# lars-frogner/Impact

Measured on AMD Instinct MI355X. Metric: voxels stepped/sec + remesh tris/sec, 512^3 grid, 1/2/4/8 MI355X, higher is better.
Workload: dtype i8 voxels, f32 SDF/mesh arithmetic, f64 moments; 1 GPU; config-2 SDF asteroid x2.05 -> 502^3 grid = 512^3 stored voxels (32768 chunks); parallelism=single GPU, voxels_per_gpu=134217728, regions=1, triangles=1813104

## Files before the change

impact_amd/csrc/ivx_api.hip:

```cpp
#include <algorithm>
#include <array>
#include <functional>
#include <cmath>
#include <atomic>
#include <chrono>
#include <cstring>
#include <limits>
#include <map>
#include <unordered_map>
#include <new>
#include <vector>

#include <type_traits>

#include <dlfcn.h>

#include "ivx_internal.hpp"

static thread_local char g_error[512] = "";

void ivx_set_error(const char* fmt, ...) {
    va_list ap;
    va_start(ap, fmt);
    vsnprintf(g_error, sizeof(g_error), fmt, ap);
// ... 86 lines not shown
            block_release(g->mesh_block);
            g->mesh_block = nullptr;
        }
    }
}
int mesh_pool_assign(ivx_grid* const* grids, size_t n, const size_t* vcaps, const size_t* icaps, const size_t* scaps) {
    if (n == 0) return IVX_OK;
    auto up = [](size_t b) { return (b + 255) & ~(size_t)255; };
    size_t total = 0;
    for (size_t i = 0; i < n; ++i) total += 2 * up(vcaps[i] * 12) + up(vcaps[i] * 16) + up(icaps[i] * 4) + up(icaps[i] * 8) + up(scaps[i] * sizeof(ivx_submesh));
    ivx_block* blk = new (std::nothrow) ivx_block();
    IVX_REQUIRE(blk, IVX_ERR_CAPACITY, "mesh buffers: out of host memory");
    blk->dev = blk->pinned = nullptr;
    blk->refs = 0;
    if (hipMalloc(&blk->dev, total) != hipSuccess) {
        delete blk;
        ivx_set_error("mesh buffers: device allocation of %zu bytes for %zu objects failed", total, n);
        return IVX_ERR_HIP;
    }
    char* b = static_cast<char*>(blk->dev);
    for (size_t i = 0; i < n; ++i) {
        ivx_grid* g = grids[i];
        mesh_group_free(g, 1u), mesh_group_free(g, 2u), mesh_group_free(g, 4u);
        auto take = [&](auto*& p, size_t bytes) {
            p = reinterpret_cast<std::remove_reference_t<decltype(p)>>(b);
            b += up(bytes);
        };
        take(g->positions, vcaps[i] * 12), take(g->normals, vcaps[i] * 12), take(g->vertex_materials, vcaps[i] * 16);
        take(g->indices, icaps[i] * 4), take(g->index_materials, icaps[i] * 8), take(g->submeshes, scaps[i] * sizeof(ivx_submesh));
        g->vcap = vcaps[i], g->icap = icaps[i], g->scap = scaps[i];
        g->mesh_block = blk;
        g->mesh_pooled = 7u;
        g->mesh_generation += 1;
        blk->refs += 1;
    }
    return IVX_OK;
}

static int mesh_arena_mode() {
    static const int m = [] {
        const char* e = getenv("IVX_MESH_ARENA");
        return e ? atoi(e) : 0;
    }();
    return m;
}
static int ensure_mesh_block(ivx_grid* g, size_t nv, size_t ni) {
    if (nv <= g->vcap && ni <= g->icap) return IVX_OK;
    IVX_HIP_CHECK(ivx_stream_sync(g->ctx->stream));
    static const size_t phase = [] {
        const char* e = getenv("IVX_MESH_PHASE");
        return (size_t)(e ? strtoull(e, nullptr, 0) : 0ull);
    }();
    const size_t vcap = std::max(2 * nv + 4096, g->vcap * 2), icap = std::max(2 * ni + 24576, g->icap * 2);
    const size_t sizes[5] = {vcap * 12, vcap * 12, icap * 4, icap * 8, vcap * 16};
    size_t off[5], total = 0;
    for (int k = 0; k < 5; ++k) {
        total = (total + (2u << 20) - 1) & ~(size_t)((2u << 20) - 1);
        off[k] = total + (size_t)k * phase;
        total = off[k] + sizes[k];
    }
    mesh_group_free(g, 1u), mesh_group_free(g, 2u);
    g->vcap = g->icap = 0;
    ivx_block* blk = new (std::nothrow) ivx_block();
    IVX_REQUIRE(blk, IVX_ERR_CAPACITY, "mesh buffers: out of host memory");
    blk->dev = blk->pinned = nullptr;
    blk->refs = 1;
    if ((mesh_arena_mode() == 2 ? hipExtMallocWithFlags(&blk->dev, total, hipDeviceMallocContiguous) : hipMalloc(&blk->dev, total)) != hipSuccess) {
        delete blk;
        ivx_set_error("mesh buffers: device allocation of %zu bytes failed", total);
        return IVX_ERR_HIP;
    }
    char* b = static_cast<char*>(blk->dev);
    g->positions = reinterpret_cast<float*>(b + off[0]);
    g->normals = reinterpret_cast<float*>(b + off[1]);
    g->indices = reinterpret_cast<uint32_t*>(b + off[2]);
    g->index_materials = reinterpret_cast<uint8_t*>(b + off[3]);
    g->vertex_materials = reinterpret_cast<uint8_t*>(b + off[4]);
    g->vcap = vcap, g->icap = icap;
    if (g->mesh_block) block_release(g->mesh_block);
    g->mesh_block = blk;
    g->mesh_pooled = 3u;
    g->mesh_generation += 1;
    return IVX_OK;
}

int ensure_mesh_capacity(ivx_grid* g, size_t nv, size_t ni, size_t ns) {
    if (mesh_arena_mode())
        if (int rc = ensure_mesh_block(g, nv, ni)) return rc;
    if (nv > g->vcap || ni > g->icap || ns > g->scap) g->mesh_generation += 1;
    if (nv > g->vcap) {
        size_t cap = std::max(2 * nv + 4096, g->vcap * 2);
        mesh_group_free(g, 1u);
        g->vcap = 0;
        int rc;
        if ((rc = dev_alloc(&g->positions, cap * 3))) return rc;
        if ((rc = dev_alloc(&g->normals, cap * 3))) return rc;
        if ((rc = dev_alloc(&g->vertex_materials, cap * 16))) return rc;
        g->vcap = cap;
    }
    if (ni > g->icap) {
        size_t cap = std::max(2 * ni + 24576, g->icap * 2);
        mesh_group_free(g, 2u);
        g->icap = 0;
        int rc;
        if ((rc = dev_alloc(&g->indices, cap))) return rc;
        if ((rc = dev_alloc(&g->index_materials, cap * 8))) return rc;
        g->icap = cap;
    }
    if (ns > g->scap) {
        size_t cap = std::max(2 * ns + 64, g->scap * 2);
        mesh_group_free(g, 4u);
        g->scap = 0;
        int rc;
        if ((rc = dev_alloc(&g->submeshes, cap))) return rc;
        g->scap = cap;
    }
    return IVX_OK;
}

__global__ __launch_bounds__(256) void k_halo_pack(GridView g, uint32_t side, int8_t* __restrict__ out_sdf, uint8_t* __restrict__ out_type,
                                                   ivx_chunk_info* __restrict__ out_info) {
    const uint32_t col = blockIdx.x;
    const uint32_t tid = threadIdx.x;
    const uint32_t ci = side ? g.cx - 1 : 0u;
    const uint32_t chunk = ci * g.cy * g.cz + col;
// ... 251 lines not shown
        carve(&g->ghost_type[sd], cols * 256);
        carve(&g->ghost_info[sd], cols);
    }
    carve(&g->chunk_counts, (size_t)g->n_chunks * 2);
    carve(&g->chunk_offsets, (size_t)g->n_chunks * 3 + 8);
    carve(&g->partials, g->partial_blocks * 10 + 16);
    carve(&g->rparent, (size_t)g->n_chunks * 256);
    carve(&g->rcompid, (size_t)g->n_chunks * 256);
    carve(&g->rscalar, (size_t)64);
    carve(&g->ccl_scratch, (size_t)g->n_chunks * 2);
    carve(&g->sn_list, (size_t)g->n_chunks * 4);
    carve(&g->group_sums, (size_t)((g->n_chunks + 255u) / 256u) * (1u + IVX_SN_GROUP_WORDS) + IVX_SN_TAIL_WORDS);
    carve(&g->sn_hard, (size_t)g->n_chunks);
    carve(&g->sn_walk, (size_t)g->n_chunks * 5 + 2);
    carve(&g->dens_dev, (size_t)256);
    carve(&g->work_counts, (size_t)8);
    carve(&g->occ_part, (size_t)((g->n_chunks + 255u) / 256u) * 12 + 12);
    carve(&g->active_list, (size_t)g->n_chunks);
    carve(&g->chunk_class, (size_t)g->n_chunks);
    carve(&g->chunk_touch, (size_t)g->n_chunks);
    carve(&g->chunk_signs, (size_t)g->n_chunks * 256);
    carve(&g->kface, (size_t)g->n_chunks * 1024);
    carve(&g->chunk_moments, (size_t)g->n_chunks * 10);
    return arena_bytes;
}
static int grid_new(ivx_ctx* c, const uint32_t cc[3], float voxel_extent, uint32_t x_chunk_offset, uint32_t global_x_chunks, ivx_grid** out) {
    IVX_REQUIRE(c && cc && out, IVX_ERR_INVALID, "ivx_grid_create: null argument");
    *out = nullptr;
    IVX_REQUIRE(cc[0] > 0 && cc[1] > 0 && cc[2] > 0, IVX_ERR_INVALID, "ivx_grid_create: empty chunk grid");
    IVX_REQUIRE(voxel_extent > 0.0f, IVX_ERR_INVALID, "ivx_grid_create: voxel extent must be positive");
    const uint64_t n64 = (uint64_t)cc[0] * cc[1] * cc[2];
    IVX_REQUIRE(n64 <= (1u << 24), IVX_ERR_CAPACITY, "ivx_grid_create: more than 2^24 chunks");
    ivx_grid* g = new (std::nothrow) ivx_grid();
    IVX_REQUIRE(g, IVX_ERR_CAPACITY, "ivx_grid_create: out of host memory");
    memset(g, 0, sizeof(*g));
    g->scratch_dirty = IVX_SCRATCH_REGIONS;
    g->ctx = c;
    for (int d = 0; d < 3; ++d) g->cc[d] = cc[d];
    g->n_chunks = (uint32_t)n64;
    g->n_vox = (size_t)n64 * IVX_CHUNK_VOXELS;
    g->extent = voxel_extent;
    g->x_off = x_chunk_offset;
    g->gx = global_x_chunks ? global_x_chunks : cc[0];
    g->partial_blocks = 2048;
    *out = g;
    return IVX_OK;
}

static void ivx_block_release(ivx_block* b) { block_release(b); }

int ivx_grid_create(ivx_ctx* c, const uint32_t cc[3], float voxel_extent, uint32_t x_chunk_offset, uint32_t global_x_chunks, ivx_grid** out) {
    ivx_grid* g = nullptr;
    int rc = grid_new(c, cc, voxel_extent, x_chunk_offset, global_x_chunks, &g);
    if (rc) return rc;
    IVX_HIP_CHECK(hipSetDevice(c->device));
    const size_t arena_bytes = grid_carve(g, nullptr);
    char* arena = nullptr;
    if (hipMalloc(reinterpret_cast<void**>(&arena), arena_bytes) != hipSuccess) {
        ivx_set_error("ivx_grid_create: device allocation of %zu bytes failed", arena_bytes);
        delete g;
        return IVX_ERR_HIP;
    }
    g->arena = arena;
    (void)grid_carve(g, arena);
    if (ivx_memset_async(g->info, 0, sizeof(ivx_chunk_info) * g->n_chunks, c->stream) != hipSuccess ||
        ivx_memset_async(g->work_counts, 0, 8 * sizeof(uint32_t), c->stream) != hipSuccess) {
        ivx_set_error("ivx_grid_create: memset failed");
// ... 3215 lines not shown
```

impact_amd/csrc/ivx_internal.hpp:

```cpp
#pragma once
#include <hip/hip_runtime.h>

#include <cstdarg>
#include <cstdint>
#include <cstdio>
#include <cstring>

#include "../../include/impact_voxel_hip.h"
#include "many.hpp"

static inline hipError_t ivx_memset_async(void* p, int v, size_t n, hipStream_t s) {
    (void)ivx_many_break();
    return hipMemsetAsync(p, v, n, s);
}
static inline hipError_t ivx_memcpy_async(void* d, const void* src, size_t n, hipMemcpyKind k, hipStream_t s) {
    (void)ivx_many_break();
    return hipMemcpyAsync(d, src, n, k, s);
}
static inline hipError_t ivx_stream_sync(hipStream_t s) {
    (void)ivx_many_break();
    return hipStreamSynchronize(s);
}
static inline hipError_t ivx_memcpy_sync(void* d, const void* src, size_t n, hipMemcpyKind k) {
    (void)ivx_many_break();
    return hipMemcpy(d, src, n, k);
}
static inline hipError_t ivx_event_record(hipEvent_t e, hipStream_t s) {
    (void)ivx_many_break();
// ... 104 lines not shown
    uint16_t* chunk_signs;
    uint8_t* chunk_touch;
    double* chunk_moments;
    uint32_t last_active;
    int planes_compact;
    int signs_current;
    uint8_t signs_type;
    int active_list_stale;
    int regions_labelled_locally;
    struct ivx_edit_state* edit;
    uint32_t post1_needs_box[12];
    const uint32_t* post1_needs_touched;
    uint32_t* post1_needs_out;
    int early_needs_on;
    uint32_t* post1_needs_early;
    uint32_t* post1_needs_counter;
    uint32_t* post1_needs_bell;
    uint32_t post1_needs_seq;
    const uint32_t* gather_copy_src;
    uint32_t* gather_copy_dst;
    uint32_t gather_copy_words;
    uint64_t gather_flush_id;
    int gather_launched;
    int sn_tail_zero;
    int needs_current;
    uint32_t stage_timing_off;
    float* dens_call;
    float* dens_dev;
    float dens_host[256];
    void* dev_scratch;
    size_t dev_scratch_bytes;
    ivx_sdf_processed_node* prog_nodes;
    uint32_t prog_n, prog_cap, prog_stack;
    uint32_t prog_shape[3];
    float prog_center[3];
    uint8_t prog_type;
    uint8_t prog_noise;
    uint32_t vt_n, vt_seed;
    float vt_noise_freq, vt_type_freq;
    uint32_t eval_len[3];
    int eval_len_valid, eval_len_pending;
    int has_dens;
    double* moments_dev;
    uint32_t* samp_len;
    void* samp_ops;
    int ahead_on, ahead_pending, ahead_wanted, ahead_unordered_ok, shadow_sel, alt_eval_dirty, ahead_events_ready;
// ... 129 lines not shown
    if (x_part == IVX_XPART_ALL) return false;
    const bool face = (ci == 0u && g.ghost_sdf[0] != nullptr) || (ci + 1u == g.cx && g.ghost_sdf[1] != nullptr);
    return face != (x_part == IVX_XPART_FACES);
}
#endif

#define IVX_LIST_CHUNK(w) ((w) & 0xFFFFFFu)
#define IVX_LIST_KIND(w) (((w) >> 24) & 3u)
#define IVX_LIST_GEN(w) (((w) >> 26) & 3u)
#define IVX_LIST_EXPOSED(w) (((w) >> 28) & 1u)

static inline uint32_t ivx_list_grid(const ivx_grid* g) {
    uint32_t n = g->last_active ? g->last_active + g->last_active / 8u + 64u : (uint32_t)g->ctx->n_cu * 32u;
    const uint32_t lo = (g->n_chunks + 255u) / 256u;
    if (n > g->n_chunks) n = g->n_chunks;
    return n < lo ? lo : n;
}

static inline bool ivx_has_interior_planes(const ivx_grid* g) { return (int)g->cc[0] - (g->has_ghost[0] ? 1 : 0) - (g->has_ghost[1] ? 1 : 0) > 0; }
static inline uint32_t* ivx_wc(const ivx_grid* g) { return g->work_counts + g->wc_cur; }
static inline void ivx_planes_touched(ivx_grid* g) {
    g->signs_current = 0;
    g->needs_current = 0;
}
#define IVX_SCRATCH_EVAL_ROLL 8u
#define IVX_SCRATCH_REGIONS 1u
#define IVX_SCRATCH_SN 2u
#define IVX_SN_TAIL_WORDS 288u
#define IVX_SN_GROUP_WORDS 32u
#define IVX_SCRATCH_EVAL 4u

static inline GridView ivx_view(const ivx_grid* g) {
    GridView v;
    v.cx = g->cc[0];
    v.cy = g->cc[1];
    v.cz = g->cc[2];
    v.sdf = g->sdf;
    v.type = g->type;
    v.signs = g->chunk_signs;
    v.kface = g->kface;
#ifdef IVX_WG_TRACE
    v.trace = reinterpret_cast<unsigned long long*>(g->chunk_moments);
#endif
    v.info = g->info;
    for (int s = 0; s < 2; ++s) {
        if (g->has_ghost[s] && g->ghost_ext[s]) {
// ... 90 lines not shown
```

impact_amd/csrc/sn_roles.hpp:

```cpp
#pragma once
#include "ivx_internal.hpp"

namespace ivx_roles {
namespace sn {


constexpr int G = 18, NROWS = 324, NCROWS = 289, NCUBES = 4913;
constexpr int RS = 24, TILE_BYTES = NROWS * RS;
constexpr uint32_t VPC = 864;
__device__ __forceinline__ int tix(int a, int b, int c) { return (a * G + b) * RS + 3 + c; }

__device__ __forceinline__ uint32_t opaque(uint32_t x) {
    asm volatile("" : "+v"(x));
    return x;
}
struct V3 {
    float x, y, z;
};
__device__ __forceinline__ V3 mk(float x, float y, float z) { return V3{x, y, z}; }
__device__ __forceinline__ V3 add(V3 a, V3 b) { return {a.x + b.x, a.y + b.y, a.z + b.z}; }
__device__ __forceinline__ V3 sub(V3 a, V3 b) { return {a.x - b.x, a.y - b.y, a.z - b.z}; }
__device__ __forceinline__ V3 mul(V3 a, V3 b) { return {a.x * b.x, a.y * b.y, a.z * b.z}; }
__device__ __forceinline__ V3 scale(V3 a, float s) { return {a.x * s, a.y * s, a.z * s}; }
__device__ __forceinline__ float len3(V3 a) { return sqrtf((a.x * a.x + a.y * a.y) + a.z * a.z); }
// ... 1032 lines not shown
    if ((s_rec[16] & 0xFFu) == KIND_NONUNIFORM) upper[1] -= 1;
    if ((s_rec[14] & 0xFFu) == KIND_NONUNIFORM) upper[2] -= 1;
}

#ifndef IVX_EMIT_ST_PER_CU
#define IVX_EMIT_ST_PER_CU 5
#endif
static inline uint32_t ivx_emit_grid(const ivx_grid* g, uint32_t n_entries, uint32_t per_cu = 4u) {
    const uint32_t resident = (uint32_t)g->ctx->n_cu * per_cu;
    return n_entries < resident ? (n_entries ? n_entries : 1u) : resident;
}
static inline uint32_t ivx_emit_general_grid(const ivx_grid* g, uint32_t n_entries) {
    const uint32_t cap = (uint32_t)g->ctx->n_cu * 2u;
    return n_entries < cap ? (n_entries ? n_entries : 1u) : cap;
}

#define IVX_MESH_ST(p, v) __builtin_nontemporal_store((v), (p))
template <bool SLOTS, bool ST = false>
__device__ __forceinline__ void role_sn_emit(uint32_t bid, uint32_t nb, SnParams p, float* __restrict__ positions, float* __restrict__ normals,
                                                 uint32_t* __restrict__ indices, unsigned long long* __restrict__ imats, ivx_submesh* __restrict__ submeshes,
                                                 const uint32_t* __restrict__ emit_count, const uint4* __restrict__ emit_items, uint32_t vcap, uint32_t icap,
                                                 uint32_t scap, const uint32_t* __restrict__ slots, uint32_t* __restrict__ hard_count,
                                                 uint32_t* __restrict__ hard_list, uint32_t* __restrict__ cursor, SnWalk walk = SnWalk{nullptr, nullptr, nullptr, 0u},
                                                 uint32_t walk_len = 0u) {
    __shared__ uint16_t s_quad[3 * VPC];
    __shared__ __attribute__((aligned(16))) uint8_t s_sd[TILE_BYTES];
    __shared__ __attribute__((aligned(16))) uint8_t s_ty[ST ? 16 : TILE_BYTES];
    __shared__ uint32_t s_neg2[2][NROWS];
    __shared__ uint32_t s_vrow[NCROWS];
    __shared__ uint16_t s_qrow[NCROWS];
    __shared__ uint2 s_qbits[NCROWS];
    __shared__ uint32_t s_nq;
    __shared__ uint16_t s_surf[VPC];
    __shared__ float s_vpos[3][VPC];
    __shared__ uint8_t s_vsm[ST ? 4 : VPC];
    __shared__ uint32_t s_wsum[4];
    __shared__ uint32_t s_hard;
    __shared__ uint32_t s_rec[27];
    __shared__ uint32_t s_ticket[5];
    __shared__ float s_rcount[13];
    const GridView& g = p.g;
    const uint32_t tid = threadIdx.x;
    if (tid >= 1u && tid < 13u) s_rcount[tid] = 1.0f / (float)tid;
    const uint32_t n_emit = emit_count[0];
    constexpr uint32_t NONE = 0xFFFFFFFFu;
    const uint32_t walk_front = walk.items ? walk.count[0] : 0u;
    uint32_t li = NONE, li_next = bid, li_prev = NONE;
    if (li_next >= n_emit) return;
    uint4 item = make_uint4(0u, 0u, 0u, 0u), item_next;
    if (walk.items) {
        const uint32_t w = bid < walk_front ? bid : walk_len - 1u - (bid - walk_front);
        item_next = walk.items[w];
        li_next = walk.li[w];
    } else {
        item_next = emit_items[li_next];
    }
    int upper[3] = {G - 1, G - 1, G - 1};
    uint32_t info_w = 0u;
    uint32_t buf = 0u;
    bool from_ticket = false;
    constexpr uint32_t TK = 192u;
    for (;;) {
    const bool have = li != NONE;
    const uint32_t* s_neg = s_neg2[buf];
    const uint32_t chunk = item.x, voff = item.y, ioff = item.z;
    const uint32_t icount = (item.w >> 16) * 6u;
    const uint32_t slot = have ? (SLOTS ? slots[li] : li) : 0u;
    const bool fits = have && !((size_t)voff + (item.w & 0xFFFFu) > vcap || (size_t)ioff + icount > icap || slot >= scap);
    const bool large = fits && (item.w & 0xFFFFu) > VPC;
    const uint32_t vcount = (fits && !large) ? (item.w & 0xFFFFu) : 0u;
    const int ck = chunk % g.cz, cj = (chunk / g.cz) % g.cy, ci = chunk / (g.cz * g.cy);
    if (have) IVX_T(g, li, 0);
    if (tid == 0 && fits) {
        const uint32_t cflags = (info_w >> 16) & 0xFFu;
        ivx_submesh sm;
        sm.chunk_indices[0] = (uint32_t)ci + p.x_off;
        sm.chunk_indices[1] = (uint32_t)cj;
        sm.chunk_indices[2] = (uint32_t)ck;
        sm.index_offset = ioff;
        sm.index_count = icount;
        for (int a = 0; a < 2; ++a)
            for (int b = 0; b < 2; ++b)
                for (int c = 0; c < 2; ++c)
                    sm.is_obscured_from_direction[a][b][c] =
                        (((cflags >> (3 * a)) & 1u) && ((cflags >> (3 * b + 1)) & 1u) && ((cflags >> (3 * c + 2)) & 1u)) ? 1u : 0u;
        sm.vertex_offset = voff;
        sm.vertex_count = item.w & 0xFFFFu;
        sm.reserved = 0;
        submeshes[slot] = sm;
    }
    __syncthreads();
    if (have) IVX_T(g, li, 1);
    if (from_ticket) {
        li_next = (uint32_t)__builtin_amdgcn_readfirstlane((int)s_ticket[0]);
        item_next = make_uint4((uint32_t)__builtin_amdgcn_readfirstlane((int)s_ticket[1]), (uint32_t)__builtin_amdgcn_readfirstlane((int)s_ticket[2]),
                               (uint32_t)__builtin_amdgcn_readfirstlane((int)s_ticket[3]), (uint32_t)__builtin_amdgcn_readfirstlane((int)s_ticket[4]));
    }
    const bool have_next = li_next < n_emit;
    bool other_type = false;
    if constexpr (ST) {
        if (tid < 64u) {
            const uint32_t w = tid < 27u ? s_rec[tid] : 0u;
            other_type = __builtin_amdgcn_ballot_w64((w & 0xFFu) == KIND_UNIFORM && (w >> 24) != p.single_type) != 0ull;
        }
    }
    if (tid == 0) {
        if (li_prev != NONE && s_hard) hard_list[atomicAdd(hard_count, 1u)] = li_prev;
        s_hard = (large || other_type) ? 1u : 0u;
    }

    uint32_t ticket = 0u;
    if (tid == TK && have_next) ticket = nb + 8u * atomicAdd(cursor + 32u * (bid & 7u), 1u) + (bid & 7u);
    TileLoads T;
    if (have_next) tile_issue<ST>(g, item_next.x, T, tid);
    uint4 drawn = make_uint4(0u, 0u, 0u, 0u);
    uint32_t drawn_li = 0u;
    {
        uint32_t vb[2] = {0, 0}, nq[2] = {0, 0};
        const int r0 = 2 * (int)opaque(tid);
        for (int q = 0; q < 2; ++q) {
            const int cr = r0 + q;
            if (cr < NCROWS) {
                uint32_t qx, qy, qz;
                cube_row_bits(s_neg, cr / 17, cr % 17, upper, vb[q], qx, qy, qz);
                nq[q] = __popc(qx) + __popc(qy) + __popc(qz);
                s_qbits[cr] = make_uint2(qx | (qy << 17), (qy >> 15) | (qz << 2));
            }
        }
        uint32_t total;
        const uint32_t pre = block_prefix<false>((__popc(vb[0]) + __popc(vb[1])) | ((nq[0] + nq[1]) << 16), s_wsum, tid, total);
        uint32_t base = pre & 0xFFFFu, qb = pre >> 16;
// ... 139 lines not shown
            const int rb = ab == 1 ? 0 : (ab == 17 ? 1 : 17), rc = ac == 1 ? 0 : (ac == 17 ? 1 : 17);
            const int kb = ab == 1 ? 1 : 0, kc = ac == 1 ? 1 : 0;
            const uint32_t v1 = vertex_of(s_vrow[cr], k), v2 = vertex_of(s_vrow[cr - rb], k - kb), v3 = vertex_of(s_vrow[cr - rc], k - kc),
                           v4 = vertex_of(s_vrow[cr - rb - rc], k - kb - kc);
            const V3 q1 = mk(s_vpos[0][v1], s_vpos[1][v1], s_vpos[2][v1]), q2 = mk(s_vpos[0][v2], s_vpos[1][v2], s_vpos[2][v2]);
            const V3 q3 = mk(s_vpos[0][v3], s_vpos[1][v3], s_vpos[2][v3]), q4 = mk(s_vpos[0][v4], s_vpos[1][v4], s_vpos[2][v4]);
            const uint32_t b1 = ST ? p.single_type : s_vsm[v1], b2 = ST ? b1 : s_vsm[v2], b3 = ST ? b1 : s_vsm[v3], b4 = ST ? b1 : s_vsm[v4];
            uint32_t quad[6];
            const V3 e14 = sub(q1, q4), e23 = sub(q2, q3);
            const float sq14 = (e14.x * e14.x + e14.y * e14.y) + e14.z * e14.z, sq23 = (e23.x * e23.x + e23.y * e23.y) + e23.z * e23.z;
            bool first = sq14 < sq23;
            if (__builtin_amdgcn_ballot_w64(first) != 0ull) first = sqrtf(sq14) < sqrtf(sq23);
            if (first) {
                if (negative_face) { quad[0] = v1; quad[1] = v4; quad[2] = v2; quad[3] = v1; quad[4] = v3; quad[5] = v4; }
                else { quad[0] = v1; quad[1] = v2; quad[2] = v4; quad[3] = v1; quad[4] = v4; quad[5] = v3; }
            } else if (negative_face) { quad[0] = v2; quad[1] = v3; quad[2] = v4; quad[3] = v2; quad[4] = v1; quad[5] = v3; }
            else { quad[0] = v2; quad[1] = v4; quad[2] = v3; quad[3] = v2; quad[4] = v3; quad[5] = v1; }
            if (q_live) {
                const size_t io = (size_t)ioff + (size_t)q * 6;
#pragma unroll
                for (int t = 0; t < 6; ++t) IVX_MESH_ST(indices + io + t, voff + quad[t]);
                if (!(b1 == b2 && b1 == b3 && b1 == b4)) s_hard = 1u;
            }
            const uint32_t rem3 = 3u * min(n_quads - q0, 64u);
            uint4* imw = reinterpret_cast<uint4*>(imats + (size_t)ioff + (size_t)q0 * 6);
#pragma unroll
            for (int jx = 0; jx < 3; ++jx) {
                const uint32_t x = lane + 64u * (uint32_t)jx;
                const uint32_t src = (x * 171u) >> 9;
                const uint32_t bm = (uint32_t)__builtin_amdgcn_ds_bpermute((int)(src << 2), (int)b1);
                if (x < rem3) {
                    uint32_t* w_ = reinterpret_cast<uint32_t*>(imw + x);
                    IVX_MESH_ST(w_, bm), IVX_MESH_ST(w_ + 1, 1u), IVX_MESH_ST(w_ + 2, bm), IVX_MESH_ST(w_ + 3, 1u);
                }
            }
        }
    }
    if (tid == TK && have_next) {
        s_ticket[0] = ticket < n_emit ? drawn_li : NONE;
        s_ticket[1] = drawn.x, s_ticket[2] = drawn.y, s_ticket[3] = drawn.z, s_ticket[4] = drawn.w;
    }
    if (have) IVX_T(g, li, 4);

    if (have_next) {
        tile_finish<ST>(g, item_next.x, T, s_rec, s_sd, s_ty, s_neg2[buf ^ 1u], tid, upper);
        info_w = s_rec[13];
    }
    if (have) IVX_T(g, li, 5);
    if (!have_next) break;
    li_prev = li;
    li = li_next;
    item = item_next;
    from_ticket = true;
    buf ^= 1u;
    }
    __syncthreads();
    if (tid == 0 && li != NONE && s_hard) hard_list[atomicAdd(hard_count, 1u)] = li;
}

template <bool SLOTS>
__device__ __forceinline__ void role_sn_emit_general(uint32_t bid, uint32_t nb, SnParams p, float* __restrict__ positions, float* __restrict__ normals,
                                                 uint32_t* __restrict__ indices, unsigned long long* __restrict__ imats,
                                                 uint4* __restrict__ vmats, ivx_submesh* __restrict__ submeshes, const uint32_t* __restrict__ emit_count,
                                                 const uint4* __restrict__ emit_items, uint32_t vcap, uint32_t icap, uint32_t scap,
                                                 const uint32_t* __restrict__ slots, const uint32_t* __restrict__ hard_count,
                                                 const uint32_t* __restrict__ hard_list) {
    __shared__ uint16_t s_quad[768];
    __shared__ __attribute__((aligned(16))) uint8_t s_sd[TILE_BYTES];
    __shared__ __attribute__((aligned(16))) uint8_t s_ty[TILE_BYTES];
    __shared__ uint32_t s_neg[NROWS];
    __shared__ uint32_t s_vrow[NCROWS];
    __shared__ uint16_t s_surf[NCUBES];
    __shared__ float s_vpos[3][VPC];
    __shared__ uint8_t s_vsm[VPC];
    __shared__ uint32_t s_wsum[4];
    const GridView& g = p.g;
    const uint32_t tid = threadIdx.x;
    const uint32_t n_emit = emit_count[0];
    const uint32_t n_hard = hard_count[0] < n_emit ? hard_count[0] : n_emit;
    for (uint32_t hi = bid; hi < n_hard; hi += nb) {
// ... 244 lines not shown
```

impact_amd/csrc/step_fused.hip:

```cpp
#include "ccl_roles.hpp"
#include "sn_roles.hpp"
#include "table_roles.hpp"
#include "many.hpp"

namespace {
using namespace ivx_roles;

struct StepArgs {
    GridView g;
    float extent;
    uint32_t x_off;
    uint32_t n_chunks;
    uint32_t nb[6];
    const uint8_t* flags;
    uint8_t* labels;
    ivx_chunk_info* info;
    uint32_t* rparent;
    uint32_t* rcompid;
    uint32_t* rscalar;
    uint32_t* multi_list;
    uint32_t* ccl_group_sums;
    const uint8_t* touch;
    uint32_t* counts;
    uint32_t* sn_group_sums;
// ... 22 lines not shown
    double* moments_out;
    uint32_t* host_block;
    const uint32_t* eval_count;
    uint32_t count_run;
    uint32_t x_part;
    uint32_t seq;
    uint32_t fp_side, fp_cap;
    const uint16_t* fp_nbr;
    uint32_t* fp_count;
    uint2* fp_pairs;
    uint32_t* fp_seen;
    unsigned long long* record;
    uint32_t record_max_pairs;
    unsigned long long* record_head;
    uint32_t record_head_words;
    sn::BoxNeeds needs_box;
    const uint32_t* needs_touched;
    uint32_t* needs_out;
    uint32_t* needs_early;
    uint32_t* needs_counter;
    uint32_t* needs_bell;
    uint32_t needs_seq;
    uint32_t single_type;
    const uint32_t* copy_src;
    uint32_t* copy_dst;
    uint32_t copy_words;
};

__device__ __forceinline__ sn::SnParams sn_params(const StepArgs& a) {
    sn::SnParams p;
    p.g = a.g;
    p.extent = a.extent;
    p.x_off = a.x_off;
    p.single_type = a.single_type;
    return p;
}

__device__ __forceinline__ void step_post1_body(const StepArgs& a, uint32_t b, uint32_t) {
    __shared__ uint32_t sh_words[4 * sn::NROWS + 16];
    struct { uint32_t* par; } sh{sh_words};
    if (b < a.nb[1]) {
        role_ccl_merge_columns(b, a.nb[1], a.g, a.touch, a.rparent);
        return;
    }
    b -= a.nb[1];
    if (b < a.nb[0]) {
// ... 73 lines not shown
    b -= a.nb[2];
    if (b < a.nb[3]) {
        role_occupied_final(a.n_occ_slots, a.occ_part, a.rscalar + 16);
        return;
    }
    b -= a.nb[3];
    if (b < a.nb[4]) {
        __shared__ uint32_t s_seen[128];
        role_face_pairs(b, a.g, a.fp_side, a.labels, a.rcompid, a.fp_nbr, a.fp_count, a.fp_pairs, a.fp_cap, a.fp_seen, s_seen);
    }
}
__global__ __launch_bounds__(256) void k_step_post2(StepArgs a) { step_post2_body(a, blockIdx.x, gridDim.x); }
IVX_MANY_TWIN(k_step_post2_many, StepArgs, step_post2_body, __launch_bounds__(256))

template <bool ST>
__device__ __forceinline__ void step_emit_body(const StepArgs& a, uint32_t b, uint32_t) {
    if (b < a.nb[0]) {
        role_ccl_flatten(b, a.nb[0], a.g, a.rparent, a.multi_list , a.ccl_group_sums);
        return;
    }
    b -= a.nb[0];
    if (b < a.nb[1]) {
        sn::role_sn_emit<false, ST>(b, a.nb[1], sn_params(a), a.positions, a.normals, a.indices, a.imats, a.submeshes, a.offsets + 2 * (size_t)a.n_chunks + 2,
                                a.emit_items, a.vcap, a.icap, a.scap, nullptr, a.hard_count, a.hard_list, a.hard_count + 32, a.walk, a.n_chunks);
        return;
    }
    b -= a.nb[1];
    if (b < a.nb[2]) {
        role_step_record(a.rscalar, a.fp_count, a.fp_pairs, a.offsets + 2 * (size_t)a.n_chunks, a.moments_out, a.x_off, a.record_max_pairs, a.record);
        if (a.record_head) {
            __syncthreads();
            for (uint32_t i = threadIdx.x; i < a.record_head_words; i += 256u) a.record_head[i] = a.record[i];
        }
        if (threadIdx.x < 64u) role_result_gather(a.rscalar, a.offsets + 2 * (size_t)a.n_chunks, a.moments_out, a.work_count, a.eval_count, a.host_block, false, 0u);
    }
}
template <bool ST>
__global__ __launch_bounds__(256) __attribute__((amdgpu_waves_per_eu(ST ? IVX_EMIT_ST_PER_CU : 4, ST ? IVX_EMIT_ST_PER_CU : 4))) void k_step_emit(StepArgs a) { step_emit_body<ST>(a, blockIdx.x, gridDim.x); }
IVX_MANY_TWIN(k_step_emit_many, StepArgs, step_emit_body<false>, __launch_bounds__(256) __attribute__((amdgpu_waves_per_eu(4, 4))))

__device__ __forceinline__ void step_assign_body(const StepArgs& a, uint32_t b, uint32_t) {
    if (b < a.nb[0]) {
        role_ccl_assign<true>(b, a.nb[0], a.g, a.rparent, a.multi_list , a.ccl_group_sums, a.nb[0], a.rcompid, a.rscalar);
        return;
    }
    sn::role_sn_emit_general<false>(b - a.nb[0], a.nb[1], sn_params(a), a.positions, a.normals, a.indices, a.imats, a.vmats, a.submeshes,
                                    a.offsets + 2 * (size_t)a.n_chunks + 2, a.emit_items, a.vcap, a.icap, a.scap, nullptr, a.hard_count, a.hard_list);
}
__global__ __launch_bounds__(256) __attribute__((amdgpu_waves_per_eu(4, 4))) void k_step_assign(StepArgs a) { step_assign_body(a, blockIdx.x, gridDim.x); }
IVX_MANY_TWIN(k_step_assign_many, StepArgs, step_assign_body, __launch_bounds__(256) __attribute__((amdgpu_waves_per_eu(4, 4))))

__device__ __forceinline__ void step_gather_body(const StepArgs& a, uint32_t, uint32_t) {
    role_result_gather(a.rscalar, a.offsets + 2 * (size_t)a.n_chunks, a.moments_out, a.work_count, a.eval_count, a.host_block, false, 0u);
    for (uint32_t i0 = threadIdx.x; i0 < a.copy_words; i0 += 512u) {
        uint32_t v[8];
#pragma unroll
        for (uint32_t q = 0; q < 8u; ++q) v[q] = i0 + 64u * q < a.copy_words ? a.copy_src[i0 + 64u * q] : 0u;
#pragma unroll
        for (uint32_t q = 0; q < 8u; ++q)
            if (i0 + 64u * q < a.copy_words) a.copy_dst[i0 + 64u * q] = v[q];
    }
    __threadfence_system();
    if (threadIdx.x == 0u) __hip_atomic_store(a.host_block + 63, a.seq, __ATOMIC_RELEASE, __HIP_MEMORY_SCOPE_SYSTEM);
}
__global__ __launch_bounds__(64) void k_step_gather(StepArgs a) { step_gather_body(a, 0u, 1u); }
IVX_MANY_TWIN(k_step_gather_many, StepArgs, step_gather_body, __launch_bounds__(64))
IVX_MANY_LAUNCHER(many_post1, k_step_post1_many, StepArgs, 256)
IVX_MANY_LAUNCHER(many_post2, k_step_post2_many, StepArgs, 256)
// ... 136 lines not shown
    const uint32_t groups = (g->n_chunks + 255u) / 256u;
    if (stages & IVX_STAGE_REGIONS) {
        a.nb[0] = g->n_chunks < 64u ? g->n_chunks : 64u;
        const uint32_t want = g->n_chunks / 16u;
        a.nb[5] = want < 8u ? (g->n_chunks < 8u ? g->n_chunks : 8u) : (want > 128u ? 128u : want);
    }
    if (stages & IVX_STAGE_REMESH) a.nb[1] = groups;
    if (stages & IVX_STAGE_INERTIA) {
        a.nb[2] = 1;
        a.n_partials = groups < (uint32_t)g->partial_blocks ? groups : (uint32_t)g->partial_blocks;
    }
    if (stages & IVX_STAGE_OCCUPIED) a.nb[3] = 1;
    const uint32_t total = a.nb[0] + a.nb[1] + a.nb[2] + a.nb[3] + a.nb[4] + a.nb[5];
    if (total == 0) return IVX_OK;
    if (!ivx_many_try(g->ctx, g, IVX_MK_POST2, total, a)) IVX_KLAUNCH(k_step_post2, dim3(total), dim3(256), 0, g->ctx->stream, a);
    IVX_HIP_CHECK(hipGetLastError());
    return IVX_OK;
}

int ivx_launch_step_emit(ivx_grid* g, uint32_t stages, bool general_in_assign, void* slab_record, bool record_has_pairs) {
    StepArgs a = make_args(g);
    const bool single_type = g->signs_current && !g->has_ghost[0] && !g->has_ghost[1] && !ivx_many_recording();
    a.single_type = g->signs_type;
    if (stages & IVX_STAGE_REGIONS) a.nb[0] = (g->n_chunks + 255u) / 256u;
    if (stages & IVX_STAGE_REMESH) {
        a.nb[1] = sn::ivx_emit_grid(g, g->n_chunks, single_type ? IVX_EMIT_ST_PER_CU : 4u);
        g->sn_tail_zero = 0;
    }
    if (slab_record) {
        face_pair_args(a, g, record_has_pairs ? reinterpret_cast<const uint16_t*>(g->pairs_dev)  : nullptr);
        a.record = static_cast<unsigned long long*>(slab_record);
        a.record_max_pairs = IVX_MAX_FACE_PAIRS;
        a.record_head = g->record_head_copy;
        a.record_head_words = g->record_head_words;
        a.nb[2] = 1;
    }
    const uint32_t total = a.nb[0] + a.nb[1] + a.nb[2];
    if (total == 0) return IVX_OK;
    if (single_type) IVX_KLAUNCH(k_step_emit<true>, dim3(total), dim3(256), 0, g->ctx->stream, a);
    else if (!ivx_many_try(g->ctx, g, IVX_MK_EMIT, total, a)) IVX_KLAUNCH(k_step_emit<false>, dim3(total), dim3(256), 0, g->ctx->stream, a);
    IVX_HIP_CHECK(hipGetLastError());
    if ((stages & IVX_STAGE_REMESH) && !general_in_assign) return ivx_launch_sn_emit_general(g);
    return IVX_OK;
}

bool ivx_step_assign_fits(const ivx_grid* g) { return (g->n_chunks + 255u) / 256u <= ASSIGN_MAX_GROUPS; }

int ivx_launch_step_assign(ivx_grid* g, bool with_mesher_general, bool with_ccl) {
    StepArgs a = make_args(g);
    a.nb[0] = with_ccl ? (g->n_chunks + 255u) / 256u : 0u;
    a.nb[1] = with_mesher_general ? sn::ivx_emit_general_grid(g, g->n_chunks) : 0u;
    if (a.nb[0] + a.nb[1] == 0u) return IVX_OK;
    if (!ivx_many_try(g->ctx, g, IVX_MK_ASSIGN, a.nb[0] + a.nb[1], a)) IVX_KLAUNCH(k_step_assign, dim3(a.nb[0] + a.nb[1]), dim3(256), 0, g->ctx->stream, a);
    IVX_HIP_CHECK(hipGetLastError());
    return IVX_OK;
}

int ivx_launch_step_gather(ivx_grid* g) {
    StepArgs a = make_args(g);
    a.seq = ++g->result_seq;
    a.copy_src = g->gather_copy_src, a.copy_dst = g->gather_copy_dst, a.copy_words = g->gather_copy_words;
    g->gather_copy_words = 0;
    if (!ivx_many_try(g->ctx, g, IVX_MK_GATHER, 1u, a)) IVX_KLAUNCH(k_step_gather, dim3(1), dim3(64), 0, g->ctx->stream, a);
    IVX_HIP_CHECK(hipGetLastError());
    return IVX_OK;
}

#ifdef IVX_WG_TRACE
extern "C" int ivx_debug_exact_trace(unsigned long long* out512) {
    return hipMemcpyFromSymbol(out512, HIP_SYMBOL(ivx_exact_trace_buf), 512 * sizeof(unsigned long long)) == hipSuccess ? 0 : -1;
}
#endif
```

impact_amd/csrc/surface_nets.hip:

```cpp
#include "sn_roles.hpp"
#include "many.hpp"

namespace {
using namespace ivx_roles::sn;

__global__ __launch_bounds__(256) void k_sn_count(SnParams p, uint32_t* __restrict__ counts, uint32_t* __restrict__ group_sums,
                                                  const uint32_t* __restrict__ work_counts, const uint32_t* __restrict__ active_list, uint32_t run) {
    __shared__ uint32_t s_rows[4 * NROWS];
    role_sn_count_waves(blockIdx.x, gridDim.x, p, counts, group_sums, work_counts, active_list, s_rows, run);
}
__global__ __launch_bounds__(256) void k_sn_scan(uint32_t n_chunks, const uint32_t* __restrict__ counts, const uint32_t* __restrict__ group_sums,
                                                 uint32_t* __restrict__ offsets, uint32_t* __restrict__ ranks, uint4* __restrict__ emit_items) {
    role_sn_scan(blockIdx.x, gridDim.x, n_chunks, counts, group_sums, offsets, ranks, emit_items);
}
template <bool SLOTS>
__global__ __launch_bounds__(256) __attribute__((amdgpu_waves_per_eu(4, 4))) void k_sn_emit(SnParams p, float* __restrict__ positions, float* __restrict__ normals,
                                                 uint32_t* __restrict__ indices, unsigned long long* __restrict__ imats, ivx_submesh* __restrict__ submeshes,
                                                 const uint32_t* __restrict__ emit_count, const uint4* __restrict__ emit_items, uint32_t vcap, uint32_t icap,
                                                 uint32_t scap, const uint32_t* __restrict__ slots, uint32_t* __restrict__ hard_count,
                                                 uint32_t* __restrict__ hard_list, uint32_t* __restrict__ cursor) {
    role_sn_emit<SLOTS>(blockIdx.x, gridDim.x, p, positions, normals, indices, imats, submeshes, emit_count, emit_items, vcap, icap, scap, slots, hard_count, hard_list,
                        cursor);
}
template <bool SLOTS>
__global__ __launch_bounds__(256) __attribute__((amdgpu_waves_per_eu(4, 4))) void k_sn_emit_general(SnParams p, float* __restrict__ positions, float* __restrict__ normals,
                                                 uint32_t* __restrict__ indices, unsigned long long* __restrict__ imats,
                                                 uint4* __restrict__ vmats, ivx_submesh* __restrict__ submeshes, const uint32_t* __restrict__ emit_count,
                                                 const uint4* __restrict__ emit_items, uint32_t vcap, uint32_t icap, uint32_t scap,
                                                 const uint32_t* __restrict__ slots, const uint32_t* __restrict__ hard_count,
                                                 const uint32_t* __restrict__ hard_list) {
    role_sn_emit_general<SLOTS>(blockIdx.x, gridDim.x, p, positions, normals, indices, imats, vmats, submeshes, emit_count, emit_items, vcap, icap, scap, slots,
                                hard_count, hard_list);
}

__global__ __launch_bounds__(256) void k_box_mesh_needs(SnParams p, BoxNeeds bx, const uint32_t* __restrict__ touched, const uint32_t* __restrict__ list,
                                                        uint32_t* __restrict__ out) {
    __shared__ uint32_t s_lds[NROWS + 2];
    role_box_mesh_needs(blockIdx.x, p, bx, touched, list, out, s_lds);
}

struct SnEmitArgs {
    SnParams p;
    float* positions;
    float* normals;
    uint32_t* indices;
    unsigned long long* imats;
    uint4* vmats;
    ivx_submesh* submeshes;
    const uint32_t* emit_count;
    const uint4* emit_items;
    const uint32_t* slots;
    uint32_t* hard_count;
    uint32_t* hard_list;
// ... 135 lines not shown
}
int ivx_launch_list_mesh_needs(ivx_grid* g, uint32_t n, const uint32_t* d_list, uint32_t* d_out) {
    if (n == 0) return IVX_OK;
    BoxNeeds bx;
    memset(&bx, 0, sizeof(bx));
    bx.b_cc[0] = bx.b_cc[1] = bx.b_cc[2] = 1u;
    IVX_KLAUNCH(k_box_mesh_needs, dim3(n), dim3(256), 0, g->ctx->stream, make_params(g), bx, nullptr, d_list, d_out);
    IVX_HIP_CHECK(hipGetLastError());
    return IVX_OK;
}

int ivx_launch_sn_scan(ivx_grid* g) {
    IVX_KLAUNCH(k_sn_scan, dim3((g->n_chunks + 255u) / 256u), dim3(256), 0, g->ctx->stream, g->n_chunks, g->chunk_counts,
                       g->group_sums + (g->n_chunks + 255u) / 256u,
                       g->chunk_offsets, g->chunk_offsets + 2 * (size_t)g->n_chunks + 4, reinterpret_cast<uint4*>(g->sn_list));
    IVX_HIP_CHECK(hipGetLastError());
    return IVX_OK;
}

uint32_t* ivx_sn_hard_count(ivx_grid* g) { return g->group_sums + (1u + IVX_SN_GROUP_WORDS) * (size_t)((g->n_chunks + 255u) / 256u); }

int ivx_launch_sn_emit(ivx_grid* g) {
    g->sn_tail_zero = 0;
    IVX_HIP_CHECK(ivx_memset_async(ivx_sn_hard_count(g), 0, IVX_SN_TAIL_WORDS * sizeof(uint32_t), g->ctx->stream));
    const uint32_t blocks = ivx_emit_grid(g, g->n_chunks);
    IVX_KLAUNCH(k_sn_emit<false>, dim3(blocks), dim3(256), 0, g->ctx->stream, make_params(g), g->positions, g->normals, g->indices,
                       reinterpret_cast<unsigned long long*>(g->index_materials), g->submeshes,
                       g->chunk_offsets + 2 * (size_t)g->n_chunks + 2, reinterpret_cast<const uint4*>(g->sn_list), (uint32_t)g->vcap, (uint32_t)g->icap,
                       (uint32_t)g->scap, nullptr, ivx_sn_hard_count(g), g->sn_hard, ivx_sn_hard_count(g) + 32);
    IVX_HIP_CHECK(hipGetLastError());
    return ivx_launch_sn_emit_general(g);
}

int ivx_launch_sn_emit_general(ivx_grid* g) {
    IVX_KLAUNCH(k_sn_emit_general<false>, dim3(ivx_emit_general_grid(g, g->n_chunks)), dim3(256), 0, g->ctx->stream, make_params(g), g->positions, g->normals,
                       g->indices, reinterpret_cast<unsigned long long*>(g->index_materials), reinterpret_cast<uint4*>(g->vertex_materials), g->submeshes,
                       g->chunk_offsets + 2 * (size_t)g->n_chunks + 2, reinterpret_cast<const uint4*>(g->sn_list), (uint32_t)g->vcap, (uint32_t)g->icap,
                       (uint32_t)g->scap, nullptr, ivx_sn_hard_count(g), g->sn_hard);
    IVX_HIP_CHECK(hipGetLastError());
    return IVX_OK;
}

int ivx_launch_sn_emit_list(ivx_grid* g, uint32_t n_records, const uint32_t* d_count, const void* d_records, const uint32_t* d_slots, uint32_t n_patch,
                            const void* d_patch_entries, const uint32_t* d_patch_slots) {
    if (n_records == 0) return IVX_OK;
    if (!g->sn_tail_zero && !ivx_many_zero(g->ctx, g, ivx_sn_hard_count(g), IVX_SN_TAIL_WORDS * sizeof(uint32_t))) {
        (void)ivx_many_break();
        IVX_HIP_CHECK(ivx_memset_async(ivx_sn_hard_count(g), 0, IVX_SN_TAIL_WORDS * sizeof(uint32_t), g->ctx->stream));
    }
    g->sn_tail_zero = 1;
    SnEmitArgs a;
    memset(&a, 0, sizeof(a));
    a.p = make_params(g), a.positions = g->positions, a.normals = g->normals, a.indices = g->indices;
    a.imats = reinterpret_cast<unsigned long long*>(g->index_materials), a.vmats = reinterpret_cast<uint4*>(g->vertex_materials), a.submeshes = g->submeshes;
    a.emit_count = d_count, a.emit_items = reinterpret_cast<const uint4*>(d_records), a.slots = d_slots, a.hard_count = ivx_sn_hard_count(g), a.hard_list = g->sn_hard;
    a.cursor = ivx_sn_hard_count(g) + 1, a.vcap = (uint32_t)g->vcap, a.icap = (uint32_t)g->icap, a.scap = (uint32_t)g->scap;
    a.n_patch = n_patch, a.patch_entries = static_cast<const ivx_submesh*>(d_patch_entries), a.patch_slots = d_patch_slots;
    const uint32_t b_main = ivx_emit_grid(g, n_records), b_gen = ivx_emit_general_grid(g, n_records);
    if (!ivx_many_try(g->ctx, g, IVX_MK_SN_EMIT_SLOTS, b_main, a)) IVX_KLAUNCH(k_sn_emit_slots, dim3(b_main), dim3(256), 0, g->ctx->stream, a);
    IVX_HIP_CHECK(hipGetLastError());
    if (!ivx_many_try(g->ctx, g, IVX_MK_SN_EMIT_GENERAL_SLOTS, b_gen, a)) IVX_KLAUNCH(k_sn_emit_general_slots, dim3(b_gen), dim3(256), 0, g->ctx->stream, a);
    IVX_HIP_CHECK(hipGetLastError());
    return IVX_OK;
}
```

Baseline: 844.6 billion voxels/s.

## Skip rewriting constant index materials in single-type remesh across steps

Adds a device-side watermark recording how much of the index-material buffer is already filled with the single material type. In the single-type fused emit path, quads whose index range lies below that watermark skip writing index materials. A later kernel raises the watermark from the current totals, or resets it when an other-type chunk appears. The aim is to cut redundant per-step write bandwidth to index_materials, at the cost of invalidation bookkeeping whenever buffers are reallocated or other emit paths run.

```diff
diff --git a/impact_amd/csrc/ivx_api.hip b/impact_amd/csrc/ivx_api.hip
--- a/impact_amd/csrc/ivx_api.hip
+++ b/impact_amd/csrc/ivx_api.hip
@@ -132,6 +132,7 @@
     for (size_t i = 0; i < n; ++i) {
         ivx_grid* g = grids[i];
         mesh_group_free(g, 1u), mesh_group_free(g, 2u), mesh_group_free(g, 4u);
+        ivx_imat_const_forget(g);
         auto take = [&](auto*& p, size_t bytes) {
             p = reinterpret_cast<std::remove_reference_t<decltype(p)>>(b);
             b += up(bytes);
@@ -170,6 +171,7 @@
         total = off[k] + sizes[k];
     }
     mesh_group_free(g, 1u), mesh_group_free(g, 2u);
+    ivx_imat_const_forget(g);
     g->vcap = g->icap = 0;
     ivx_block* blk = new (std::nothrow) ivx_block();
     IVX_REQUIRE(blk, IVX_ERR_CAPACITY, "mesh buffers: out of host memory");
@@ -211,6 +213,7 @@
     if (ni > g->icap) {
         size_t cap = std::max(2 * ni + 24576, g->icap * 2);
         mesh_group_free(g, 2u);
+        ivx_imat_const_forget(g);
         g->icap = 0;
         int rc;
         if ((rc = dev_alloc(&g->indices, cap))) return rc;
@@ -508,6 +511,7 @@
     carve(&g->chunk_signs, (size_t)g->n_chunks * 256);
     carve(&g->kface, (size_t)g->n_chunks * 1024);
     carve(&g->chunk_moments, (size_t)g->n_chunks * 10);
+    carve(&g->imat_const, (size_t)2);
     return arena_bytes;
 }
 static int grid_new(ivx_ctx* c, const uint32_t cc[3], float voxel_extent, uint32_t x_chunk_offset, uint32_t global_x_chunks, ivx_grid** out) {
@@ -529,6 +533,7 @@
     g->x_off = x_chunk_offset;
     g->gx = global_x_chunks ? global_x_chunks : cc[0];
     g->partial_blocks = 2048;
+    g->imat_const_type = -1;
     *out = g;
     return IVX_OK;
 }
diff --git a/impact_amd/csrc/ivx_internal.hpp b/impact_amd/csrc/ivx_internal.hpp
--- a/impact_amd/csrc/ivx_internal.hpp
+++ b/impact_amd/csrc/ivx_internal.hpp
@@ -4,6 +4,7 @@
 #include <cstdarg>
 #include <cstdint>
 #include <cstdio>
+#include <cstdlib>
 #include <cstring>
 
 #include "../../include/impact_voxel_hip.h"
@@ -154,6 +155,8 @@
     uint32_t gather_copy_words;
     uint64_t gather_flush_id;
     int gather_launched;
+    uint32_t* imat_const;
+    int imat_const_type, imat_const_valid, imat_raise_pending;
     int sn_tail_zero;
     int needs_current;
     uint32_t stage_timing_off;
@@ -329,6 +332,15 @@
 static inline void ivx_planes_touched(ivx_grid* g) {
     g->signs_current = 0;
     g->needs_current = 0;
+}
+static inline void ivx_imat_const_forget(ivx_grid* g) {
+    g->imat_const_valid = 0;
+    g->imat_const_type = -1;
+    g->imat_raise_pending = 0;
+}
+static inline bool ivx_imat_always() {
+    static const bool on = getenv("IVX_EMIT_IMAT_ALWAYS") && atoi(getenv("IVX_EMIT_IMAT_ALWAYS")) != 0;
+    return on;
 }
 #define IVX_SCRATCH_EVAL_ROLL 8u
 #define IVX_SCRATCH_REGIONS 1u
diff --git a/impact_amd/csrc/sn_roles.hpp b/impact_amd/csrc/sn_roles.hpp
--- a/impact_amd/csrc/sn_roles.hpp
+++ b/impact_amd/csrc/sn_roles.hpp
@@ -1078,7 +1078,7 @@
                                                  const uint32_t* __restrict__ emit_count, const uint4* __restrict__ emit_items, uint32_t vcap, uint32_t icap,
                                                  uint32_t scap, const uint32_t* __restrict__ slots, uint32_t* __restrict__ hard_count,
                                                  uint32_t* __restrict__ hard_list, uint32_t* __restrict__ cursor, SnWalk walk = SnWalk{nullptr, nullptr, nullptr, 0u},
-                                                 uint32_t walk_len = 0u) {
+                                                 uint32_t walk_len = 0u, uint32_t* __restrict__ imat_const = nullptr) {
     __shared__ uint16_t s_quad[3 * VPC];
     __shared__ __attribute__((aligned(16))) uint8_t s_sd[TILE_BYTES];
     __shared__ __attribute__((aligned(16))) uint8_t s_ty[ST ? 16 : TILE_BYTES];
@@ -1099,6 +1099,7 @@
     const uint32_t tid = threadIdx.x;
     if (tid >= 1u && tid < 13u) s_rcount[tid] = 1.0f / (float)tid;
     const uint32_t n_emit = emit_count[0];
+    const uint32_t imat_upto = (ST && imat_const) ? imat_const[0] : 0u;
     constexpr uint32_t NONE = 0xFFFFFFFFu;
     const uint32_t walk_front = walk.items ? walk.count[0] : 0u;
     uint32_t li = NONE, li_next = bid, li_prev = NONE;
@@ -1125,6 +1126,7 @@
     const bool fits = have && !((size_t)voff + (item.w & 0xFFFFu) > vcap || (size_t)ioff + icount > icap || slot >= scap);
     const bool large = fits && (item.w & 0xFFFFu) > VPC;
     const uint32_t vcount = (fits && !large) ? (item.w & 0xFFFFu) : 0u;
+    const bool imat_keep = ST && (size_t)ioff + icount <= imat_upto;
     const int ck = chunk % g.cz, cj = (chunk / g.cz) % g.cy, ci = chunk / (g.cz * g.cy);
     if (have) IVX_T(g, li, 0);
     if (tid == 0 && fits) {
@@ -1163,6 +1165,7 @@
     if (tid == 0) {
         if (li_prev != NONE && s_hard) hard_list[atomicAdd(hard_count, 1u)] = li_prev;
         s_hard = (large || other_type) ? 1u : 0u;
+        if (ST && imat_const && have && other_type) imat_const[1] = 1u;
     }
 
     uint32_t ticket = 0u;
@@ -1348,6 +1351,7 @@
                 for (int t = 0; t < 6; ++t) IVX_MESH_ST(indices + io + t, voff + quad[t]);
                 if (!(b1 == b2 && b1 == b3 && b1 == b4)) s_hard = 1u;
             }
+            if (imat_keep) continue;
             const uint32_t rem3 = 3u * min(n_quads - q0, 64u);
             uint4* imw = reinterpret_cast<uint4*>(imats + (size_t)ioff + (size_t)q0 * 6);
 #pragma unroll
@@ -1382,6 +1386,16 @@
     }
     __syncthreads();
     if (tid == 0 && li != NONE && s_hard) hard_list[atomicAdd(hard_count, 1u)] = li;
+}
+
+__device__ __forceinline__ void imat_const_raise(uint32_t* __restrict__ imat_const, const uint32_t* __restrict__ totals, uint32_t vcap, uint32_t icap,
+                                                 uint32_t scap) {
+    if (imat_const[1]) {
+        imat_const[0] = 0u;
+        imat_const[1] = 0u;
+    } else if (totals[0] <= vcap && totals[1] <= icap && totals[2] <= scap && totals[1] > imat_const[0]) {
+        imat_const[0] = totals[1];
+    }
 }
 
 template <bool SLOTS>
diff --git a/impact_amd/csrc/step_fused.hip b/impact_amd/csrc/step_fused.hip
--- a/impact_amd/csrc/step_fused.hip
+++ b/impact_amd/csrc/step_fused.hip
@@ -68,6 +68,8 @@
     uint32_t* needs_bell;
     uint32_t needs_seq;
     uint32_t single_type;
+    uint32_t imat_raise;
+    uint32_t* imat_const;
     const uint32_t* copy_src;
     uint32_t* copy_dst;
     uint32_t copy_words;
@@ -187,7 +189,8 @@
     b -= a.nb[0];
     if (b < a.nb[1]) {
         sn::role_sn_emit<false, ST>(b, a.nb[1], sn_params(a), a.positions, a.normals, a.indices, a.imats, a.submeshes, a.offsets + 2 * (size_t)a.n_chunks + 2,
-                                a.emit_items, a.vcap, a.icap, a.scap, nullptr, a.hard_count, a.hard_list, a.hard_count + 32, a.walk, a.n_chunks);
+                                a.emit_items, a.vcap, a.icap, a.scap, nullptr, a.hard_count, a.hard_list, a.hard_count + 32, a.walk, a.n_chunks,
+                                    ST ? a.imat_const : nullptr);
         return;
     }
     b -= a.nb[1];
@@ -209,6 +212,7 @@
         role_ccl_assign<true>(b, a.nb[0], a.g, a.rparent, a.multi_list , a.ccl_group_sums, a.nb[0], a.rcompid, a.rscalar);
         return;
     }
+    if (a.imat_raise && b == a.nb[0] && threadIdx.x == 0u) sn::imat_const_raise(a.imat_const, a.offsets + 2 * (size_t)a.n_chunks, a.vcap, a.icap, a.scap);
     sn::role_sn_emit_general<false>(b - a.nb[0], a.nb[1], sn_params(a), a.positions, a.normals, a.indices, a.imats, a.vmats, a.submeshes,
                                     a.offsets + 2 * (size_t)a.n_chunks + 2, a.emit_items, a.vcap, a.icap, a.scap, nullptr, a.hard_count, a.hard_list);
 }
@@ -391,6 +395,18 @@
     StepArgs a = make_args(g);
     const bool single_type = g->signs_current && !g->has_ghost[0] && !g->has_ghost[1] && !ivx_many_recording();
     a.single_type = g->signs_type;
+    g->imat_raise_pending = 0;
+    if ((stages & IVX_STAGE_REMESH) && single_type && !ivx_imat_always()) {
+        if (!g->imat_const_valid || g->imat_const_type != (int)g->signs_type) {
+            IVX_HIP_CHECK(ivx_memset_async(g->imat_const, 0, 2 * sizeof(uint32_t), g->ctx->stream));
+            g->imat_const_valid = 1;
+            g->imat_const_type = (int)g->signs_type;
+        }
+        a.imat_const = g->imat_const;
+        g->imat_raise_pending = 1;
+    } else if (stages & IVX_STAGE_REMESH) {
+        ivx_imat_const_forget(g);
+    }
     if (stages & IVX_STAGE_REGIONS) a.nb[0] = (g->n_chunks + 255u) / 256u;
     if (stages & IVX_STAGE_REMESH) {
         a.nb[1] = sn::ivx_emit_grid(g, g->n_chunks, single_type ? IVX_EMIT_ST_PER_CU : 4u);
@@ -419,6 +435,10 @@
     StepArgs a = make_args(g);
     a.nb[0] = with_ccl ? (g->n_chunks + 255u) / 256u : 0u;
     a.nb[1] = with_mesher_general ? sn::ivx_emit_general_grid(g, g->n_chunks) : 0u;
+    if (with_mesher_general && g->imat_raise_pending) {
+        a.imat_raise = 1u, a.imat_const = g->imat_const;
+        g->imat_raise_pending = 0;
+    }
     if (a.nb[0] + a.nb[1] == 0u) return IVX_OK;
     if (!ivx_many_try(g->ctx, g, IVX_MK_ASSIGN, a.nb[0] + a.nb[1], a)) IVX_KLAUNCH(k_step_assign, dim3(a.nb[0] + a.nb[1]), dim3(256), 0, g->ctx->stream, a);
     IVX_HIP_CHECK(hipGetLastError());
diff --git a/impact_amd/csrc/surface_nets.hip b/impact_amd/csrc/surface_nets.hip
--- a/impact_amd/csrc/surface_nets.hip
+++ b/impact_amd/csrc/surface_nets.hip
@@ -28,7 +28,8 @@
                                                  uint4* __restrict__ vmats, ivx_submesh* __restrict__ submeshes, const uint32_t* __restrict__ emit_count,
                                                  const uint4* __restrict__ emit_items, uint32_t vcap, uint32_t icap, uint32_t scap,
                                                  const uint32_t* __restrict__ slots, const uint32_t* __restrict__ hard_count,
-                                                 const uint32_t* __restrict__ hard_list) {
+                                                 const uint32_t* __restrict__ hard_list, uint32_t* __restrict__ imat_raise) {
+    if (imat_raise && blockIdx.x == 0u && threadIdx.x == 0u) imat_const_raise(imat_raise, emit_count - 2, vcap, icap, scap);
     role_sn_emit_general<SLOTS>(blockIdx.x, gridDim.x, p, positions, normals, indices, imats, vmats, submeshes, emit_count, emit_items, vcap, icap, scap, slots,
                                 hard_count, hard_list);
 }
@@ -210,6 +211,7 @@
 
 int ivx_launch_sn_emit(ivx_grid* g) {
     g->sn_tail_zero = 0;
+    ivx_imat_const_forget(g);
     IVX_HIP_CHECK(ivx_memset_async(ivx_sn_hard_count(g), 0, IVX_SN_TAIL_WORDS * sizeof(uint32_t), g->ctx->stream));
     const uint32_t blocks = ivx_emit_grid(g, g->n_chunks);
     IVX_KLAUNCH(k_sn_emit<false>, dim3(blocks), dim3(256), 0, g->ctx->stream, make_params(g), g->positions, g->normals, g->indices,
@@ -221,10 +223,12 @@
 }
 
 int ivx_launch_sn_emit_general(ivx_grid* g) {
+    uint32_t* imat_raise = g->imat_raise_pending ? g->imat_const : nullptr;
+    g->imat_raise_pending = 0;
     IVX_KLAUNCH(k_sn_emit_general<false>, dim3(ivx_emit_general_grid(g, g->n_chunks)), dim3(256), 0, g->ctx->stream, make_params(g), g->positions, g->normals,
                        g->indices, reinterpret_cast<unsigned long long*>(g->index_materials), reinterpret_cast<uint4*>(g->vertex_materials), g->submeshes,
                        g->chunk_offsets + 2 * (size_t)g->n_chunks + 2, reinterpret_cast<const uint4*>(g->sn_list), (uint32_t)g->vcap, (uint32_t)g->icap,
-                       (uint32_t)g->scap, nullptr, ivx_sn_hard_count(g), g->sn_hard);
+                       (uint32_t)g->scap, nullptr, ivx_sn_hard_count(g), g->sn_hard, imat_raise);
     IVX_HIP_CHECK(hipGetLastError());
     return IVX_OK;
 }
@@ -232,6 +236,7 @@
 int ivx_launch_sn_emit_list(ivx_grid* g, uint32_t n_records, const uint32_t* d_count, const void* d_records, const uint32_t* d_slots, uint32_t n_patch,
                             const void* d_patch_entries, const uint32_t* d_patch_slots) {
     if (n_records == 0) return IVX_OK;
+    ivx_imat_const_forget(g);
     if (!g->sn_tail_zero && !ivx_many_zero(g->ctx, g, ivx_sn_hard_count(g), IVX_SN_TAIL_WORDS * sizeof(uint32_t))) {
         (void)ivx_many_break();
         IVX_HIP_CHECK(ivx_memset_async(ivx_sn_hard_count(g), 0, IVX_SN_TAIL_WORDS * sizeof(uint32_t), g->ctx->stream));
```

New measurement: 842.2 billion voxels/s (median of 2 runs). About the same (-0.3%).
